# Rongjiehuang/FastDiff

Measured on AMD Instinct MI355X. Metric: real-time factor (audio-sec/wall-sec), N=4 reverse steps, 80x864 mel, higher is better.
Workload: dtype f32 results; 2-piece fp16 operands (22 bit) on fp16 MFMA, fp32 accumulate; GEMM as Winograd F(2,3); exact-fp32 twin; 1 GPU; BASELINE configs[1]: LJSpeech shape, batch=8 x 80x864 mel per GPU, N=4, HIP kernels + hipGraph sampler; batch_per_gpu=8, frames=864, reverse_steps=4, graph=True, weights=random init seed 1234 (no checkpoint offline), world_size=1, gpus_visible=1, oversubscribed=False

## Files before the change

fastdiff_amd/csrc/fd_kernels_kp.hip:

```cpp
#include "fd_kernels_common.h"

namespace fdk_fast {

constexpr int KPF_VALID = 48, KPF_LDI = 68, KPF_LDH = 66;

struct KpFrontW {
    const float *in_pack[fd::NBLK], *in_b[fd::NBLK];
    const float *res_pack[fd::NBLK][6], *res_b[fd::NBLK][6];
};

__global__ void __launch_bounds__(256, 2) k_kp_front(const float *__restrict__ mel, float *__restrict__ hout, KpFrontW w,
                                                     const float *__restrict__ noise, const StepParams *params, int sampler,
                                                     int B, int T, const int *__restrict__ run_if, const int *__restrict__ lens)
{
    __shared__ float xin[fd::COND * KPF_LDI];
    if (run_if && *run_if == 0) return;
    __shared__ float h0[fd::HID * KPF_LDH];
    __shared__ float hA[fd::HID * KPF_LDH];
    __shared__ float hB[fd::HID * KPF_LDH];
    const int blk = blockIdx.z, b = blockIdx.y, t0 = blockIdx.x * KPF_VALID;
    const int Tb = frames_of(lens, b, T);
    if (t0 >= Tb) return;
    const int tid = threadIdx.x, lane = tid & 63, wave = tid >> 6, l31 = lane & 31, hi = lane >> 5;
    const int mt = wave & 1, nt = wave >> 1;
    const int step = sampler ? params->step_idx : 0;
    const float *nz = noise + (((int64_t)step * (sampler > 1 ? B / sampler : B) + b) * fd::NBLK + blk) * fd::COND;
    {
        constexpr int TOTAL = fd::COND * KPF_LDI, NK = (TOTAL + 255) / 256;
        float v[NK];
        const float *src = mel + (int64_t)b * fd::COND * T;
#pragma unroll
        for (int k = 0; k < NK; ++k) {
            const int idx = k * 256 + tid, ci = idx / KPF_LDI, cc = idx - ci * KPF_LDI, t = t0 - 10 + cc;
            v[k] = (idx < TOTAL && t >= 0 && t < Tb) ? src[(int64_t)ci * T + t] + nz[ci] : 0.0f;
        }
#pragma unroll
        for (int k = 0; k < NK; ++k) {
            const int idx = k * 256 + tid;
            if (idx < TOTAL) xin[idx] = v[k];
        }
        if (tid < 128) {
            const int row = tid >> 1, col = (tid & 1) ? KPF_LDH - 1 : 0;
            h0[row * KPF_LDH + col] = 0.0f; hA[row * KPF_LDH + col] = 0.0f; hB[row * KPF_LDH + col] = 0.0f;
        }
    }
    __syncthreads();
    const int c = nt * 32 + l31;
    const int t = t0 - 8 + c;
    const bool inside = (t >= 0 && t < Tb);
    {
        const float4 *pa = reinterpret_cast<const float4 *>(w.in_pack[blk]) + (int64_t)mt * 50 * 64 + lane;
        f32x16 acc;
#pragma unroll
        for (int r = 0; r < 16; ++r) acc[r] = w.in_b[blk][mt * 32 + drow(r, hi)];
#pragma unroll 5
        for (int s4 = 0; s4 < 50; ++s4) {
            const float4 a4 = pa[s4 * 64];
#pragma unroll
            for (int r = 0; r < 4; ++r) {
                const int kk = 8 * s4 + 2 * r, tap = kk / fd::COND, ci = kk % fd::COND + hi;
                acc = mfma32(f4c(a4, r), xin[ci * KPF_LDI + c + tap], acc);
            }
        }
#pragma unroll
        for (int r = 0; r < 16; ++r) h0[(mt * 32 + drow(r, hi)) * KPF_LDH + c + 1] = inside ? lrelu(acc[r], 0.1f) : 0.0f;
    }
    __syncthreads();
    const float *src = h0;
#pragma unroll 1
    for (int l = 0; l < 6; ++l) {
        float *dst = (l & 1) ? hB : hA;
        const float4 *pa = reinterpret_cast<const float4 *>(w.res_pack[blk][l]) + (int64_t)mt * 24 * 64 + lane;
        float4 wa[24];
#pragma unroll
        for (int i = 0; i < 24; ++i) wa[i] = pa[i * 64];
        f32x16 acc;
#pragma unroll
        for (int r = 0; r < 16; ++r) acc[r] = w.res_b[blk][l][mt * 32 + drow(r, hi)];
#pragma unroll
        for (int s = 0; s < 96; ++s) {
            const int tap = s >> 5, ci = ((2 * s) & 63) + hi;
            acc = mfma32(f4c(wa[s >> 2], s & 3), src[ci * KPF_LDH + c + tap], acc);
        }
        if (l < 5) {
#pragma unroll
            for (int r = 0; r < 16; ++r) dst[(mt * 32 + drow(r, hi)) * KPF_LDH + c + 1] = inside ? lrelu(acc[r], 0.1f) : 0.0f;
            __syncthreads();
            src = dst;
        } else if (inside && c >= 8 && c < 8 + KPF_VALID) {
#pragma unroll
            for (int r = 0; r < 16; ++r) {
                const int o = mt * 32 + drow(r, hi);
                hout[(((int64_t)blk * B + b) * fd::HID + o) * T + t] = lrelu(acc[r], 0.1f) + h0[o * KPF_LDH + c + 1];
            }
        }
    }
}

constexpr int KPF_XROW = 336;

struct KpFrontW2 {
    const float4 *in_pack[fd::NBLK];
    const float *in_b[fd::NBLK];
    const float4 *res_pack[fd::NBLK][6];
    const float *res_b[fd::NBLK][6];
};

__device__ __forceinline__ int kpf_off(int row, int slot) { return row * 256 + ((slot ^ (row & 15)) << 4); }

__global__ void __launch_bounds__(256, 2) k_kp_front_h2(const float *__restrict__ mel, float *__restrict__ hout, char *__restrict__ himg,
                                                        KpFrontW2 w, const float *__restrict__ noise, const StepParams *params, int sampler,
                                                        int B, int T, int R, int *__restrict__ range_flags, const int *__restrict__ lens)
{
    __shared__ __attribute__((aligned(16))) char xin[68 * KPF_XROW];
    __shared__ __attribute__((aligned(16))) char hA[66 * 256];
    __shared__ __attribute__((aligned(16))) char hB[66 * 256];
    const int blk = blockIdx.z, b = blockIdx.y, t0 = blockIdx.x * KPF_VALID;
    const int Tb = frames_of(lens, b, T);
    if (range_flags[32 + 19] | range_flags[32]) {
        if (blockIdx.x == 0 && blockIdx.y == 0 && blockIdx.z == 0 && threadIdx.x == 0) { atomicOr(range_flags + 19, 1); atomicOr(range_flags, 1); }
        return;
    }
    if (t0 > Tb) return;
    const int tid = threadIdx.x, lane = tid & 63, wave = tid >> 6, l31 = lane & 31, hi = lane >> 5;
    const int mt = wave & 1, nt = wave >> 1;
    const int step = sampler ? params->step_idx : 0;
    const float *nz = noise + (((int64_t)step * (sampler > 1 ? B / sampler : B) + b) * fd::NBLK + blk) * fd::COND;
    float mx = 0.0f;
    {
        const float *src = mel + (int64_t)b * fd::COND * T;
        float v[3][8];
#pragma unroll
        for (int k = 0; k < 3; ++k) {
            const int u = k * 256 + tid, cg = u / 68, cc = u - cg * 68, t = t0 - 10 + cc;
            const bool ok = u < 680 && t >= 0 && t < Tb;
#pragma unroll
            for (int c = 0; c < 8; ++c) v[k][c] = ok ? src[(int64_t)(cg * 8 + c) * T + t] + nz[cg * 8 + c] : 0.0f;
        }
#pragma unroll
        for (int k = 0; k < 3; ++k) {
            const int u = k * 256 + tid, cg = u / 68, cc = u - cg * 68;
            if (u < 680) {
#pragma unroll
                for (int c = 0; c < 8; ++c) mx = fmaxf(mx, fabsf(v[k][c]));
                float4 ph, pl;
                split8(v[k], ph, pl);
                *reinterpret_cast<float4 *>(xin + cc * KPF_XROW + cg * 16) = ph;
                *reinterpret_cast<float4 *>(xin + cc * KPF_XROW + 160 + cg * 16) = pl;
            }
        }
        if (tid < 64) {
            const int row = (tid & 32) ? 65 : 0, part = tid & 15;
            char *img = (tid & 16) ? hB : hA;
            *reinterpret_cast<float4 *>(img + row * 256 + part * 16) = make_float4(0.f, 0.f, 0.f, 0.f);
        }
    }
    __syncthreads();
    const int c = nt * 32 + l31;
    const int t = t0 - 8 + c;
    const bool inside = (t >= 0 && t < Tb);
    float h0v[16];
    auto store_act = [&](char *img, const f32x16 &ah, const f32x16 &al, float *keep) {
        const int row = c + 1;
#pragma unroll
        for (int j = 0; j < 4; ++j) {
            float v[4];
#pragma unroll
            for (int i = 0; i < 4; ++i) {
                v[i] = inside ? lrelu(fmaf(al[4 * j + i], GX_INV_SCALE, ah[4 * j + i]), 0.1f) : 0.0f;
                mx = fmaxf(mx, fabsf(v[i]));
                if (keep) keep[4 * j + i] = v[i];
            }
            uint2 ph, pl;
            split2(v[0], v[1], ph.x, pl.x);
            split2(v[2], v[3], ph.y, pl.y);
            *reinterpret_cast<uint2 *>(img + kpf_off(row, mt * 4 + j) + 8 * hi) = ph;
            *reinterpret_cast<uint2 *>(img + kpf_off(row, 8 + mt * 4 + j) + 8 * hi) = pl;
        }
    };
    {
        const float4 *pa = w.in_pack[blk] + (int64_t)mt * 2 * 25 * 64 + lane;
        f32x16 ah, al;
#pragma unroll
        for (int r = 0; r < 16; ++r) { ah[r] = w.in_b[blk][mt * 32 + drow(r, hi)]; al[r] = 0.0f; }
        const char *xb = xin + c * KPF_XROW + hi * 16;
#pragma unroll 5
        for (int kg = 0; kg < 25; ++kg) {
            const float4 w1 = pa[kg * 64], w2 = pa[(25 + kg) * 64];
            const int tap = (16 * kg) / fd::COND, o = ((16 * kg) % fd::COND) / 8;
            const float4 b1 = *reinterpret_cast<const float4 *>(xb + tap * KPF_XROW + o * 16);
            const float4 b2 = *reinterpret_cast<const float4 *>(xb + tap * KPF_XROW + 160 + o * 16);
            ah = mfma_f16(w1, b1, ah);
            al = mfma_f16(w1, b2, al);
            al = mfma_f16(w2, b1, al);
        }
        store_act(hA, ah, al, h0v);
    }
    __syncthreads();
    int off[3][2][4];
#pragma unroll
    for (int tap = 0; tap < 3; ++tap)
#pragma unroll
        for (int p = 0; p < 2; ++p)
#pragma unroll
            for (int k4 = 0; k4 < 4; ++k4) off[tap][p][k4] = kpf_off(c + tap, p * 8 + k4 * 2 + hi);
    float4 wa[2][12];
    auto load_w = [&](int l) {
        const float4 *pa = w.res_pack[blk][l] + (int64_t)mt * 2 * 12 * 64 + lane;
#pragma unroll
        for (int p = 0; p < 2; ++p)
#pragma unroll
            for (int kg = 0; kg < 12; ++kg) wa[p][kg] = pa[(p * 12 + kg) * 64];
    };
    load_w(0);
#pragma unroll 1
    for (int l = 0; l < 6; ++l) {
        const char *src = (l & 1) ? hB : hA;
        char *dst = (l & 1) ? hA : hB;
        f32x16 ah, al;
#pragma unroll
        for (int r = 0; r < 16; ++r) { ah[r] = w.res_b[blk][l][mt * 32 + drow(r, hi)]; al[r] = 0.0f; }
#pragma unroll
        for (int kg = 0; kg < 12; ++kg) {
            const float4 b1 = *reinterpret_cast<const float4 *>(src + off[kg >> 2][0][kg & 3]);
            const float4 b2 = *reinterpret_cast<const float4 *>(src + off[kg >> 2][1][kg & 3]);
            ah = mfma_f16(wa[0][kg], b1, ah);
            al = mfma_f16(wa[0][kg], b2, al);
            al = mfma_f16(wa[1][kg], b1, al);
        }
        __builtin_amdgcn_sched_barrier(0);
        if (l < 5) load_w(l + 1);
        __builtin_amdgcn_sched_barrier(0);
        if (l < 5) {
            store_act(dst, ah, al, nullptr);
            __syncthreads();
        } else if (t >= 0 && t < T && c >= 8 && c < 8 + KPF_VALID) {
            char *irow = himg + (((int64_t)blk * B + b) * R + (t + 1)) * 256;
            const int sw = (t + 1) & 15;
#pragma unroll
            for (int j = 0; j < 4; ++j) {
                float v[4];
#pragma unroll
                for (int i = 0; i < 4; ++i) {
                    const int r = 4 * j + i;
                    v[i] = inside ? lrelu(fmaf(al[r], GX_INV_SCALE, ah[r]), 0.1f) + h0v[r] : 0.0f;
                    mx = fmaxf(mx, fabsf(v[i]));
                    hout[(((int64_t)blk * B + b) * fd::HID + mt * 32 + drow(r, hi)) * T + t] = v[i];
                }
                if (himg) {
                    uint2 ph, pl;
                    split2(v[0], v[1], ph.x, pl.x);
                    split2(v[2], v[3], ph.y, pl.y);
                    *reinterpret_cast<uint2 *>(irow + (((mt * 4 + j) ^ sw) << 4) + 8 * hi) = ph;
                    *reinterpret_cast<uint2 *>(irow + (((8 + mt * 4 + j) ^ sw) << 4) + 8 * hi) = pl;
                }
            }
        }
    }
    if (himg) {
        char *ib = himg + ((int64_t)blk * B + b) * R * 256;
        if (blockIdx.x == 0 && tid < 16) *reinterpret_cast<float4 *>(ib + tid * 16) = make_float4(0.f, 0.f, 0.f, 0.f);
        if (blockIdx.x == gridDim.x - 1)
            for (int e = tid; e < (R - 1 - T) * 16; e += 256) *reinterpret_cast<float4 *>(ib + (T + 1) * 256 + e * 16) = make_float4(0.f, 0.f, 0.f, 0.f);
    }
    if (!(mx < GX_LIMIT)) { atomicOr(range_flags + 19, 1); atomicOr(range_flags, 1); }
}

constexpr int GEMM_CT = 4;
constexpr int GEMM_LDH = GEMM_CT * 32 + 4;
constexpr int GEMM_NCOLS = GEMM_CT * 32 + 2;
constexpr int GEMM_NK = (fd::HID * GEMM_NCOLS + 255) / 256;

#ifdef FD_GEMM_TIMING
__device__ long long fd_gdbg[64 * 4 * 4];
#endif

__global__ void __launch_bounds__(256, 2) k_kp_gemm(const float *__restrict__ h , float *__restrict__ kpack,
                                                    const float *g0, const float *g1, const float *g2, const float *gb0,
                                                    const float *gb1, const float *gb2, int B, int T, int chunks_per_utt,
                                                    int chunk_tiles, int n_items, const int *__restrict__ run_if, const int *__restrict__ lens)
{
    __shared__ float hs[2][fd::HID * GEMM_LDH];
    if (run_if && *run_if == 0) return;
    const int tid = threadIdx.x, lane = tid & 63, wave = tid >> 6, l31 = lane & 31, hi = lane >> 5;
    constexpr int XG = fd::KREC / 128;
    const int ny = B * chunks_per_utt;
    const int i0 = (int)((int64_t)blockIdx.x * n_items / gridDim.x), i1 = (int)((int64_t)(blockIdx.x + 1) * n_items / gridDim.x);
    if (i0 >= i1) return;

    struct Item { int blk, xg, b, t_begin; };
    auto decode = [&](int id) {
        Item it;
        it.blk = id / (XG * ny);
        const int rem = id - it.blk * (XG * ny);
        it.xg = rem / ny;
        const int yy = rem - it.xg * ny;
        it.b = yy / chunks_per_utt;
        it.t_begin = (yy - it.b * chunks_per_utt) * chunk_tiles * 32;
        return it;
    };
    float v[33];
    const int scol = tid & 127, srow = tid >> 7;
#define FD_GEMM_FETCH(it)                                                                                              \
    do {                                                                                                               \
        const float *hb__ = h + (((int64_t)(it).blk * B + (it).b) * fd::HID + srow) * T + ((it).t_begin - 1);          \
        const bool ok__ = ((it).t_begin - 1 + scol) >= 0 && ((it).t_begin - 1 + scol) < frames_of(lens, (it).b, T);    \
        _Pragma("unroll") for (int j = 0; j < 32; ++j) v[j] = ok__ ? hb__[(int64_t)(2 * j) * T + scol] : 0.0f;         \
        const int t2__ = (it).t_begin + 127 + (tid & 1);               \
        v[32] = (tid < 128 && t2__ < frames_of(lens, (it).b, T)) ? hb__[(int64_t)((tid >> 1) - srow) * T + 128 + (tid & 1)] : 0.0f;                \
    } while (0)
#define FD_GEMM_COMMIT(bufi)                                                                                           \
    do {                                                                                                               \
        float *hd__ = hs[bufi] + srow * GEMM_LDH + scol;                                                               \
        _Pragma("unroll") for (int j = 0; j < 32; ++j) hd__[2 * j * GEMM_LDH] = v[j];                                   \
        if (tid < 128) hs[bufi][(tid >> 1) * GEMM_LDH + 128 + (tid & 1)] = v[32];                                       \
    } while (0)

    Item cur = decode(i0);
    FD_GEMM_FETCH(cur);
    FD_GEMM_COMMIT(0);
    __syncthreads();
    float4 wb[24];
    float bias = 0.0f;
    int have_blk = -1, have_xg = -1, buf = 0;
#pragma unroll 1
    for (int i = i0; i < i1; ++i) {
        if (cur.blk != have_blk || cur.xg != have_xg) {
            const float *gp = cur.blk == 0 ? g0 : (cur.blk == 1 ? g1 : g2);
            const float *gb = cur.blk == 0 ? gb0 : (cur.blk == 1 ? gb1 : gb2);
            const int ptile = cur.xg * 4 + wave;
#pragma unroll
            for (int k = 0; k < 24; ++k) wb[k] = reinterpret_cast<const float4 *>(gp)[((int64_t)ptile * 24 + k) * 64 + lane];
            bias = gb[ptile * 32 + l31];
            have_blk = cur.blk; have_xg = cur.xg;
        }
        Item nxt = cur;
        const bool more = (i + 1 < i1);
        if (more) { nxt = decode(i + 1); FD_GEMM_FETCH(nxt); }
        const int Tb = frames_of(lens, cur.b, T);
        const int n_frames = min(Tb - cur.t_begin, chunk_tiles * 32);
        const int n_tiles = (n_frames + 31) >> 5;
        float *kout = kpack + ((int64_t)cur.blk * B + cur.b) * T * fd::KREC + (cur.xg * 4 + wave) * 32 + l31;
#pragma unroll 1
        for (int tile = 0; tile < n_tiles; ++tile) {
            f32x16 acc;
#pragma unroll
            for (int r = 0; r < 16; ++r) acc[r] = bias;
            const int hc = hi * GEMM_LDH + l31 + tile * 32;
            const int ho3[3] = {opaque(hc), opaque(hc + 1), opaque(hc + 2)};
#pragma unroll
            for (int s = 0; s < 96; ++s) {
                const int tap = s >> 5, c2 = (2 * s) & 63;
                acc = mfma32(hs[buf][ho3[tap] + c2 * GEMM_LDH], f4c(wb[s >> 2], s & 3), acc);
            }
            const int t0 = cur.t_begin + tile * 32;
            const unsigned base = (unsigned)(t0 + 4 * hi) * (unsigned)fd::KREC;
#ifdef FD_GX_NO_STORE
            if (acc[0] != 12345.678f) continue;
#endif
            if (t0 + 32 <= Tb) {
#pragma unroll
                for (int r = 0; r < 16; ++r) kout[base + (unsigned)(((r & 3) + 8 * (r >> 2)) * fd::KREC)] = acc[r];
            } else {
#pragma unroll
                for (int r = 0; r < 16; ++r)
                    if (t0 + drow(r, hi) < Tb) kout[base + (unsigned)(((r & 3) + 8 * (r >> 2)) * fd::KREC)] = acc[r];
            }
        }
        if (more) FD_GEMM_COMMIT(buf ^ 1);
        __syncthreads();
        buf ^= 1;
        cur = nxt;
    }
}

constexpr int GX_ROWS = GX_CT * 32 + 2;
constexpr int GX_WINB = GX_ROWS * GX_ROWB;
constexpr int GX_NDMA = (GX_WINB + 4095) / 4096;
constexpr int GX_BUFB = GX_NDMA * 4096;
#ifndef FD_GX_STORE_AUX
#define FD_GX_STORE_AUX 2
#endif


__global__ void __launch_bounds__(256) k_h_split(const float *__restrict__ h, unsigned *__restrict__ hx, int *__restrict__ range_flag,
                                                 int B, int T, int R, const int *__restrict__ lens)
{
    const int bb = blockIdx.y;
    const int e = blockIdx.x * 256 + threadIdx.x, cp = e / R, row = e - cp * R;
    if (cp >= 32) return;
    if (range_flag[32] != 0) {
        if (e == 0 && bb == 0) atomicOr(range_flag, 1);
        return;
    }
    const int t = row - 1;
    const bool ok = t >= 0 && t < frames_of(lens, bb % B, T);
    const float *hb = h + (int64_t)bb * fd::HID * T;
    const float a = ok ? hb[(int64_t)(2 * cp) * T + t] : 0.0f, b2 = ok ? hb[(int64_t)(2 * cp + 1) * T + t] : 0.0f;
    if (!(fmaxf(fabsf(a), fabsf(b2)) < GX_LIMIT)) atomicOr(range_flag, 1);
    const _Float16 a1 = (_Float16)a, b1 = (_Float16)b2;
    const _Float16 a2 = (_Float16)((a - (float)a1) * GX_SCALE), b3 = (_Float16)((b2 - (float)b1) * GX_SCALE);
    union { _Float16 h[2]; unsigned u; } p1, p2;
    p1.h[0] = a1; p1.h[1] = b1;
    p2.h[0] = a2; p2.h[1] = b3;
    unsigned *dst = hx + ((int64_t)bb * R + row) * 64 + (cp & 3);
    const unsigned sw = (unsigned)row & 15u, slot = (unsigned)cp >> 2;
    dst[((slot ^ sw) << 2)] = p1.u;
    dst[(((slot + 8u) ^ sw) << 2)] = p2.u;
}

typedef __attribute__((address_space(3))) void *lds_ptr_t;

struct GxItem { int blk, xg, b, chunk; };

struct GxWalk {
    static constexpr int XG = fd::KREC / 128;
    int B, chunks, ny, n_wg, w, q, base, r0, r1;
    int n_mine, left0;
    __device__ __forceinline__ GxWalk(int B_, int chunks_per_utt, int n_items, int n_wg_, int w_)
        : B(B_), chunks(chunks_per_utt), ny(B_ * chunks_per_utt), n_wg(n_wg_), w(w_)
    {
        q = (fd::NBLK * XG) / n_wg; base = q * n_wg * ny;
        const int rest = n_items - base;
        r0 = (int)((int64_t)w * rest / n_wg); r1 = (int)((int64_t)(w + 1) * rest / n_wg);
        n_mine = q * ny + (r1 - r0);
        left0 = (q > 0) ? ny : (r1 - r0);
    }
    __device__ __forceinline__ GxItem decode(int id) const
    {
        GxItem it;
        it.blk = id / (XG * ny);
        const int rem = id - it.blk * (XG * ny);
        it.xg = rem / ny;
        const int yy = rem - it.xg * ny;
        it.b = yy / chunks;
        it.chunk = yy - it.b * chunks;
        return it;
    }
    __device__ __forceinline__ GxItem first() const { return decode((q > 0) ? w * ny : base + r0); }
    __device__ __forceinline__ GxItem advance(GxItem it) const
    {
        if (++it.chunk == chunks) {
            it.chunk = 0;
            if (++it.b == B) {
                it.b = 0;
                if (++it.xg == XG) { it.xg = 0; ++it.blk; }
            }
        }
        return it;
    }
};
#define GX_WALK_NEXT(walk, cur, more, nxt, run, left)                                                                  \
    GxItem nxt = cur;                                                                                                  \
    if (more) {                                                                                                        \
        if (left > 1) nxt = (walk).advance(cur);                                                                       \
        else {                                                  \
            ++run;                                                                                                     \
            nxt = (walk).decode(run < (walk).q ? (run * (walk).n_wg + (walk).w) * (walk).ny : (walk).base + (walk).r0); \
            left = (run < (walk).q ? (walk).ny : (walk).r1 - (walk).r0) + 1;                                           \
        }                                                                                                              \
    }                                                                                                                  \
    --left

template <int ROUNDS, bool PARTIAL_LAST>
__device__ __forceinline__ void gx_window_dma(const char *src , char *lds_buf, int wave_u, int lane)
{
    const unsigned dst = (unsigned)(uintptr_t)(lds_ptr_t)(lds_buf + wave_u * 1024);
    const unsigned voff = lane * 16;
    unsigned keep;
#pragma unroll
    for (int j = 0; j < ROUNDS; ++j) {
        if (PARTIAL_LAST && j == ROUNDS - 1 && wave_u != 0) break;
        asm volatile("s_mov_b32 %0, m0\n\ts_mov_b32 m0, %3\n\ts_nop 0\n\tglobal_load_lds_dwordx4 %1, %2\n\ts_mov_b32 m0, %0"
                     : "=&s"(keep)
                     : "v"(voff), "s"(src + j * 4096), "s"(dst + j * 4096)
                     : "memory");
    }
}

__device__ __forceinline__ void gx_dma(const char *hx, char *lds_buf, const GxItem &it, int B, int R, int wave_u, int lane)
{
#ifndef FD_GX_NO_FETCH
    gx_window_dma<GX_NDMA, true>(hx + (((int64_t)it.blk * B + it.b) * R + it.chunk * (GX_CT * 32)) * GX_ROWB + wave_u * 1024, lds_buf, wave_u, lane);
#endif
}

#ifdef FD_GX_TIMING
__device__ long long fd_gxdbg[8];
#define GX_STAMP(k) do { const long long t__ = __builtin_amdgcn_s_memtime(); ph[k] += t__ - tl; tl = t__; } while (0)
#define GX_TIMING_ARGS , long long (&ph)[8], long long &tl
#define GX_TIMING_PASS , ph, tl
#else
#define GX_STAMP(k) do { } while (0)
#define GX_TIMING_ARGS
#define GX_TIMING_PASS
#endif
template <int BUF, bool FULL>
__device__ __forceinline__ void gx_item(char *lds, const GxItem &cur, bool more, const GxItem &nxt, const char *hx, float *kpack,
                                        const float4 (&wq)[2][12], const f32x16 &bias_lo, const int (&aoff)[2][12], int B, int T, int R,
                                        int wave_u, int lane, int Tb GX_TIMING_ARGS)
{
    const int l31 = lane & 31, hi = lane >> 5;
    GX_STAMP(0);
    if (more) gx_dma(hx, lds + (BUF ^ 1) * GX_BUFB, nxt, B, R, wave_u, lane);
    GX_STAMP(1);
    const int t_begin = cur.chunk * (GX_CT * 32);
    float *krow = kpack + (((int64_t)cur.blk * B + cur.b) * T + t_begin) * fd::KREC + (cur.xg * 4 + wave_u) * 32;
    const unsigned loff = (unsigned)(4 * hi) * (unsigned)fd::KREC + (unsigned)l31;
    const __amdgpu_buffer_rsrc_t rs = __builtin_amdgcn_make_buffer_rsrc(krow, 0, GX_CT * 32 * fd::KREC * 4, 0x00020000);
    const int n_tiles = max(0, min(GX_CT, (Tb - t_begin + 31) >> 5));
    const f32x16 zero = {0.f, 0.f, 0.f, 0.f, 0.f, 0.f, 0.f, 0.f, 0.f, 0.f, 0.f, 0.f, 0.f, 0.f, 0.f, 0.f};
#pragma unroll
    for (int tile = 0; tile < GX_CT; ++tile) {
        if (tile >= n_tiles) break;
        const char *hb = lds + BUF * GX_BUFB + tile * 32 * GX_ROWB;
        f32x16 acc, lo;
        float4 a1 = *reinterpret_cast<const float4 *>(hb + aoff[0][0]), a2 = *reinterpret_cast<const float4 *>(hb + aoff[1][0]);
#pragma unroll
        for (int kg = 0; kg < 12; ++kg) {
            float4 n1 = a1, n2 = a2;
            if (kg + 1 < 12) {
                n1 = *reinterpret_cast<const float4 *>(hb + aoff[0][kg + 1]);
                n2 = *reinterpret_cast<const float4 *>(hb + aoff[1][kg + 1]);
            }
            acc = mfma_f16(a1, wq[0][kg], kg == 0 ? zero : acc);
            lo = mfma_f16(a2, wq[0][kg], kg == 0 ? bias_lo : lo);
#ifndef FD_GX_PROBE_TWO_MFMA
            lo = mfma_f16(a1, wq[1][kg], lo);
#endif
            a1 = n1;
            a2 = n2;
        }
        GX_STAMP(2);
#ifdef FD_GX_NO_STORE
        if (acc[0] != 12345.678f) continue;
#endif
        if (FULL) {
#ifdef FD_GX_STORE_AUX_B0
            if (cur.blk == 0) {
#pragma unroll
                for (int r = 0; r < 16; ++r)
                    __builtin_amdgcn_raw_buffer_store_b32(__float_as_uint(fmaf(lo[r], GX_INV_SCALE, acc[r])), rs, loff * 4u,
                                                          (tile * 32 + (r & 3) + 8 * (r >> 2)) * fd::KREC * 4, FD_GX_STORE_AUX_B0);
            } else
#endif
#pragma unroll
            for (int r = 0; r < 16; ++r)
                __builtin_amdgcn_raw_buffer_store_b32(__float_as_uint(fmaf(lo[r], GX_INV_SCALE, acc[r])), rs, loff * 4u,
                                                      (tile * 32 + (r & 3) + 8 * (r >> 2)) * fd::KREC * 4, FD_GX_STORE_AUX);
        } else {
            float *kt = krow + (int64_t)tile * 32 * fd::KREC;
#pragma unroll
            for (int r = 0; r < 16; ++r)
                if (t_begin + tile * 32 + drow(r, hi) < Tb)
                    (kt + ((r & 3) + 8 * (r >> 2)) * fd::KREC)[loff] = fmaf(lo[r], GX_INV_SCALE, acc[r]);
        }
        GX_STAMP(3);
    }
    if (more) {
        if (FULL && n_tiles == 4) asm volatile("s_waitcnt vmcnt(63)" ::: "memory");
        else if (FULL && n_tiles == 3) asm volatile("s_waitcnt vmcnt(48)" ::: "memory");
        else if (FULL && n_tiles == 2) asm volatile("s_waitcnt vmcnt(32)" ::: "memory");
        else if (FULL && n_tiles == 1) asm volatile("s_waitcnt vmcnt(16)" ::: "memory");
        else asm volatile("s_waitcnt vmcnt(0)" ::: "memory");
    }
    GX_STAMP(4);
    __builtin_amdgcn_s_barrier();
    GX_STAMP(5);
}

__global__ void __launch_bounds__(256, 2) k_kp_gemm_h2(const char *__restrict__ hx , float *__restrict__ kpack,
                                                       const float4 *g0, const float4 *g1, const float4 *g2, const float *gb0,
                                                       const float *gb1, const float *gb2, const int *__restrict__ range_flag, int B,
                                                       int T, int R, int chunks_per_utt, int n_items, const int *__restrict__ lens)
{
    __shared__ __attribute__((aligned(16))) char lds[2 * GX_BUFB];
    const int tid = threadIdx.x, lane = tid & 63, l31 = lane & 31, hi = lane >> 5;
    const int wave_u = __builtin_amdgcn_readfirstlane(tid >> 6);
    if (*range_flag != 0) return;

    GxWalk walk(B, chunks_per_utt, n_items, gridDim.x, blockIdx.x);
    const int n_mine = walk.n_mine;
    if (n_mine <= 0) return;
    int run = 0, left = walk.left0;
    GxItem cur = walk.first();

    int aoff[2][12];
#pragma unroll
    for (int q = 0; q < 2; ++q)
#pragma unroll
        for (int tap = 0; tap < 3; ++tap)
#pragma unroll
            for (int k4 = 0; k4 < 4; ++k4) {
                const int row = l31 + tap;
                aoff[q][tap * 4 + k4] = row * GX_ROWB + (((q * 8 + k4 * 2 + hi) ^ (row & 15)) << 4);
            }

    gx_dma(hx, lds, cur, B, R, wave_u, lane);
    asm volatile("s_waitcnt vmcnt(0)" ::: "memory");
    __builtin_amdgcn_s_barrier();

#ifdef FD_GX_TIMING
    long long ph[8] = {0, 0, 0, 0, 0, 0, 0, 0}, tl = __builtin_amdgcn_s_memtime();
    const long long t_start = tl, r_start = __builtin_amdgcn_s_memrealtime();
#endif
    float4 wq[2][12];
    f32x16 bias_lo;
    int have_blk = -1, have_xg = -1;
#pragma unroll 1
    for (int i = 0; i < n_mine; i += 2) {
#pragma unroll
        for (int half = 0; half < 2; ++half) {
            if (half == 1 && i + 1 >= n_mine) break;
            if (cur.blk != have_blk || cur.xg != have_xg) {
                const float4 *gp = cur.blk == 0 ? g0 : (cur.blk == 1 ? g1 : g2);
                const float *gb = cur.blk == 0 ? gb0 : (cur.blk == 1 ? gb1 : gb2);
                const int ptile = cur.xg * 4 + wave_u;
#pragma unroll
                for (int q2 = 0; q2 < 2; ++q2)
#pragma unroll
                    for (int kg = 0; kg < 12; ++kg) wq[q2][kg] = gp[(((int64_t)ptile * 2 + q2) * 12 + kg) * 64 + lane];
                const float bv = gb[ptile * 32 + l31] * GX_SCALE;
#pragma unroll
                for (int r = 0; r < 16; ++r) bias_lo[r] = bv;
                have_blk = cur.blk; have_xg = cur.xg;
                __builtin_amdgcn_s_waitcnt(0x0F70);
            }
            const bool more = (i + half + 1 < n_mine);
            GX_WALK_NEXT(walk, cur, more, nxt, run, left);
            const int Tb = frames_of(lens, cur.b, T);
            const bool full = (Tb % 32 == 0) || (cur.chunk * (GX_CT * 32) + GX_CT * 32 <= Tb);
            if (half == 0) {
                if (full) gx_item<0, true>(lds, cur, more, nxt, hx, kpack, wq, bias_lo, aoff, B, T, R, wave_u, lane, Tb GX_TIMING_PASS);
                else gx_item<0, false>(lds, cur, more, nxt, hx, kpack, wq, bias_lo, aoff, B, T, R, wave_u, lane, Tb GX_TIMING_PASS);
            } else {
                if (full) gx_item<1, true>(lds, cur, more, nxt, hx, kpack, wq, bias_lo, aoff, B, T, R, wave_u, lane, Tb GX_TIMING_PASS);
                else gx_item<1, false>(lds, cur, more, nxt, hx, kpack, wq, bias_lo, aoff, B, T, R, wave_u, lane, Tb GX_TIMING_PASS);
            }
            cur = nxt;
        }
    }
#ifdef FD_GX_TIMING
    ph[6] = __builtin_amdgcn_s_memtime() - t_start;
    ph[7] = __builtin_amdgcn_s_memrealtime() - r_start;
    if (lane == 0)
        for (int k = 0; k < 8; ++k) atomicAdd((unsigned long long *)&fd_gxdbg[k], (unsigned long long)ph[k]);
#endif
}

constexpr int GW_WINB = GW_PAIRS * GW_ROWB;

__global__ void __launch_bounds__(256) k_h_wino(const float *__restrict__ h, char *__restrict__ wx, int *__restrict__ range_flag, int B, int T,
                                                int P, const int *__restrict__ lens)
{
    const int bb = blockIdx.y;
    const int e = blockIdx.x * 256 + threadIdx.x, p = e >> 3, g = e & 7;
    if (p >= P) return;
    if (range_flag[32] != 0) {
        if (e == 0 && bb == 0) atomicOr(range_flag, 1);
        return;
    }
    const int Tb = frames_of(lens, bb % B, T);
    const float *hb = h + ((int64_t)bb * fd::HID + 8 * g) * T;
    const int t1 = 2 * p;
    float d[8][4];
#pragma unroll
    for (int c = 0; c < 8; ++c) {
        const float *hc = hb + (int64_t)c * T;
        d[c][0] = (t1 - 1 >= 0 && t1 - 1 < Tb) ? hc[t1 - 1] : 0.0f;
        d[c][1] = (t1 < Tb) ? hc[t1] : 0.0f;
        d[c][2] = (t1 + 1 < Tb) ? hc[t1 + 1] : 0.0f;
        d[c][3] = (t1 + 2 < Tb) ? hc[t1 + 2] : 0.0f;
    }
    float mx = 0.0f;
    char *row = wx + ((int64_t)bb * P + p) * GW_ROWB;
    const int sw = p & 15;
#pragma unroll
    for (int j = 0; j < 4; ++j) {
        float u[8];
#pragma unroll
        for (int c = 0; c < 8; ++c) {
            u[c] = j == 0 ? d[c][0] - d[c][2] : (j == 1 ? d[c][1] + d[c][2] : (j == 2 ? d[c][2] - d[c][1] : d[c][1] - d[c][3]));
            mx = fmaxf(mx, fabsf(u[c]));
        }
        float4 ph, pl;
        split8(u, ph, pl);
        *reinterpret_cast<float4 *>(row + j * 256 + ((g ^ sw) << 4)) = ph;
        *reinterpret_cast<float4 *>(row + j * 256 + (((g + 8) ^ sw) << 4)) = pl;
    }
    if (!(mx < GX_LIMIT)) atomicOr(range_flag, 1);
}

__device__ __forceinline__ void gw_dma(const char *wx, char *lds_buf, const GxItem &it, int B, int P, int wave_u, int lane)
{
#ifndef FD_GW_NO_FETCH
    gx_window_dma<GW_WINB / 4096, false>(wx + (((int64_t)it.blk * B + it.b) * P + it.chunk * GW_PAIRS) * GW_ROWB + wave_u * 1024, lds_buf, wave_u, lane);
#endif
}

template <int BUF, bool FULL>
__device__ __forceinline__ void gw_item(char *lds, const GxItem &cur, bool more, const GxItem &nxt, const char *wx, float *kpack,
                                        const float4 (&wq)[2][16], float bias_lo, const int (&aoff)[2][4], int B, int T, int P,
                                        int wave_u, int lane, int Tb)
{
    const int l31 = lane & 31, hi = lane >> 5;
    if (more) gw_dma(wx, lds + (BUF ^ 1) * GW_WINB, nxt, B, P, wave_u, lane);
    const int t_begin = cur.chunk * (2 * GW_PAIRS);
    float *krow = kpack + (((int64_t)cur.blk * B + cur.b) * T + t_begin) * fd::KREC + (cur.xg * 4 + wave_u) * 32;
    const unsigned loff = (unsigned)(8 * hi) * (unsigned)fd::KREC + (unsigned)l31;
    const __amdgpu_buffer_rsrc_t rs = __builtin_amdgcn_make_buffer_rsrc(krow, 0, 2 * GW_PAIRS * fd::KREC * 4, 0x00020000);
    const f32x16 zero = {0.f, 0.f, 0.f, 0.f, 0.f, 0.f, 0.f, 0.f, 0.f, 0.f, 0.f, 0.f, 0.f, 0.f, 0.f, 0.f};
    const char *hb = lds + BUF * GW_WINB;
    constexpr int ORDER[4] = {1, 2, 0, 3};
    f32x16 keep, acc, lo;
#pragma unroll
    for (int r = 0; r < 16; ++r) lo[r] = bias_lo;
    float4 a1, a2;
    auto store16 = [&](int odd) {
#ifdef FD_GX_NO_STORE
        if (FULL) {
#pragma unroll
            for (int r = 0; r < 16; ++r) { const float v_ = fmaf(lo[r], GX_INV_SCALE, acc[r]); asm volatile("" :: "v"(v_)); }
            (void)rs; (void)loff;
            return;
        }
#endif
        if (FULL) {
#pragma unroll
            for (int r = 0; r < 16; ++r) {
                acc[r] = fmaf(lo[r], GX_INV_SCALE, acc[r]);
                __builtin_amdgcn_raw_buffer_store_b32(__float_as_uint(acc[r]), rs, loff * 4u, (2 * ((r & 3) + 8 * (r >> 2)) + odd) * fd::KREC * 4,
                                                      FD_GX_STORE_AUX);
            }
        } else {
#pragma unroll
            for (int r = 0; r < 16; ++r)
                if (t_begin + 2 * drow(r, hi) + odd < Tb) (krow + (2 * ((r & 3) + 8 * (r >> 2)) + odd) * fd::KREC)[loff] = fmaf(lo[r], GX_INV_SCALE, acc[r]);
        }
    };
#pragma unroll
    for (int s = 0; s < 4; ++s) {
        const int j = ORDER[s];
        a1 = *reinterpret_cast<const float4 *>(hb + aoff[0][0] + j * 256);
        a2 = *reinterpret_cast<const float4 *>(hb + aoff[1][0] + j * 256);
#pragma unroll
        for (int k4 = 0; k4 < 4; ++k4) {
            const int kg = j * 4 + k4;
            float4 n1 = a1, n2 = a2;
            if (k4 + 1 < 4) {
                n1 = *reinterpret_cast<const float4 *>(hb + aoff[0][k4 + 1] + j * 256);
                n2 = *reinterpret_cast<const float4 *>(hb + aoff[1][k4 + 1] + j * 256);
            }
            acc = mfma_f16(a1, wq[0][kg], (k4 == 0 && s == 0) ? zero : ((k4 == 0 && s == 3) ? keep : acc));
            lo = mfma_f16(a2, wq[0][kg], (k4 == 0 && s == 3) ? zero : lo);
            lo = mfma_f16(a1, wq[1][kg], lo);
            a1 = n1;
            a2 = n2;
        }
        if (s == 0) {
#pragma unroll
            for (int r = 0; r < 16; ++r) keep[r] = fmaf(lo[r], GX_INV_SCALE, acc[r]);
        } else if (s == 1) {
#pragma unroll
            for (int r = 0; r < 16; ++r) keep[r] = fmaf(2.0f, keep[r], -fmaf(lo[r], GX_INV_SCALE, acc[r]));
        } else store16(s == 3 ? 1 : 0);
    }
    if (more) {
#ifdef FD_GX_NO_STORE
        asm volatile("s_waitcnt vmcnt(0)" ::: "memory");
#else
        if (FULL) asm volatile("s_waitcnt vmcnt(32)" ::: "memory");
        else asm volatile("s_waitcnt vmcnt(0)" ::: "memory");
#endif
    }
    __builtin_amdgcn_s_barrier();
}

typedef float gw_f4 __attribute__((ext_vector_type(4)));
__device__ __forceinline__ gw_f4 mfma16_f16(const float4 &a, const float4 &b, gw_f4 c)
{
    union { float4 f; f16x8 h; } ua, ub;
    ua.f = a;
    ub.f = b;
    return __builtin_amdgcn_mfma_f32_16x16x32_f16(ua.h, ub.h, c, 0, 0, 0);
}
template <int BUF>
__device__ __forceinline__ void gw16_item(char *lds, const GxItem &cur, bool more, const GxItem &nxt, const char *wx, float *kpack,
                                          const float4 (&wq)[2][16] , const float (&bias_lo)[2],
                                          const int (&aoff)[2][2], int B, int T, int P, int wave_u, int lane, int Tb)
{
    if (more) gw_dma(wx, lds + (BUF ^ 1) * GW_WINB, nxt, B, P, wave_u, lane);
    const int t_begin = cur.chunk * (2 * GW_PAIRS);
    float *krow = kpack + (((int64_t)cur.blk * B + cur.b) * T + t_begin) * fd::KREC + (cur.xg * 4 + wave_u) * 32;
    const unsigned loff = gw16_st_lane_off(lane);
    const __amdgpu_buffer_rsrc_t rs = __builtin_amdgcn_make_buffer_rsrc(krow, 0, 2 * GW_PAIRS * fd::KREC * 4, 0x00020000);
    const gw_f4 zero = {0.f, 0.f, 0.f, 0.f};
    constexpr int ORDER[4] = {1, 2, 0, 3};
    int n_fast = 0;
    bool counted = true;
#pragma unroll
    for (int rt = 0; rt < 2; ++rt) {
        const int t0 = t_begin + 32 * rt;
        if (t0 >= Tb) continue;
        const bool whole = t0 + 32 <= Tb;
        const char *hb = lds + BUF * GW_WINB + rt * 16 * GW_ROWB;
        gw_f4 acc[2], lo[2], keep[2];
#pragma unroll
        for (int ct = 0; ct < 2; ++ct) lo[ct] = gw_f4{bias_lo[ct], bias_lo[ct], bias_lo[ct], bias_lo[ct]};
        float4 a1 = *reinterpret_cast<const float4 *>(hb + aoff[0][0] + ORDER[0] * 256);
        float4 a2 = *reinterpret_cast<const float4 *>(hb + aoff[1][0] + ORDER[0] * 256);
#ifdef FD_GW16_PIN
        __builtin_amdgcn_sched_group_barrier(0x100, 2, 0);
#endif
#pragma unroll
        for (int step = 0; step < 8; ++step) {
            const int s = step >> 1, ks = step & 1, j = ORDER[s], w = (2 * j + ks) * 2;
            float4 n1 = a1, n2 = a2;
            if (step + 1 < 8) {
                const int jn = ORDER[(step + 1) >> 1], kn = (step + 1) & 1;
                n1 = *reinterpret_cast<const float4 *>(hb + aoff[0][kn] + jn * 256);
                n2 = *reinterpret_cast<const float4 *>(hb + aoff[1][kn] + jn * 256);
            }
            const bool m3 = (step == 6);
            acc[0] = mfma16_f16(a1, wq[0][w], step == 0 ? zero : (m3 ? keep[0] : acc[0]));
            lo[0] = mfma16_f16(a2, wq[0][w], m3 ? zero : lo[0]);
            acc[1] = mfma16_f16(a1, wq[0][w + 1], step == 0 ? zero : (m3 ? keep[1] : acc[1]));
            lo[1] = mfma16_f16(a2, wq[0][w + 1], m3 ? zero : lo[1]);
            lo[0] = mfma16_f16(a1, wq[1][w], lo[0]);
            lo[1] = mfma16_f16(a1, wq[1][w + 1], lo[1]);
            a1 = n1;
            a2 = n2;
#ifdef FD_GW16_PIN
            if (step + 1 < 8) __builtin_amdgcn_sched_group_barrier(0x100, 2, 0);
            __builtin_amdgcn_sched_group_barrier(0x008, 6, 0);
#endif
            if (ks == 0) continue;
            if (s == 0) {
#pragma unroll
                for (int ct = 0; ct < 2; ++ct)
#pragma unroll
                    for (int i = 0; i < 4; ++i) keep[ct][i] = fmaf(lo[ct][i], GX_INV_SCALE, acc[ct][i]);
            } else if (s == 1) {
#pragma unroll
                for (int ct = 0; ct < 2; ++ct)
#pragma unroll
                    for (int i = 0; i < 4; ++i) keep[ct][i] = fmaf(2.0f, keep[ct][i], -fmaf(lo[ct][i], GX_INV_SCALE, acc[ct][i]));
            } else {
                const int odd = s == 3 ? 1 : 0;
                float v[2][4];
#pragma unroll
                for (int ct = 0; ct < 2; ++ct)
#pragma unroll
                    for (int i = 0; i < 4; ++i) v[ct][i] = fmaf(lo[ct][i], GX_INV_SCALE, acc[ct][i]);
                if (whole) {
#pragma unroll
                    for (int i = 0; i < 4; ++i) {
                        const auto x = __builtin_amdgcn_permlane16_swap(__float_as_uint(v[0][i]), __float_as_uint(v[1][i]), false, false);
#pragma unroll
                        for (int part = 0; part < 2; ++part)
                            __builtin_amdgcn_raw_buffer_store_b32(x[part], rs, loff * 4u, gw16_st_row_off(rt, part, i, odd) * 4, FD_GX_STORE_AUX);
                    }
                } else {
#pragma unroll
                    for (int ct = 0; ct < 2; ++ct)
#pragma unroll
                        for (int i = 0; i < 4; ++i) {
                            const int f = 2 * (16 * rt + gw16_d_pair(lane, i)) + odd;
                            if (t_begin + f < Tb) krow[f * fd::KREC + gw16_d_pos(lane, ct)] = v[ct][i];
                        }
                }
            }
        }
        if (whole) ++n_fast;
        else counted = false;
    }
    if (more) {
        if (counted && n_fast == 2) asm volatile("s_waitcnt vmcnt(32)" ::: "memory");
        else if (counted && n_fast == 1) asm volatile("s_waitcnt vmcnt(16)" ::: "memory");
        else asm volatile("s_waitcnt vmcnt(0)" ::: "memory");
    }
    __builtin_amdgcn_s_barrier();
}

#ifdef FD_GW_CLOCK
__device__ long long fd_gwclk[2];
#endif
template <int TILE>
__global__ void __launch_bounds__(256, 2) k_kp_gemm_w(const char *__restrict__ wx , float *__restrict__ kpack,
                                                      const float4 *g0, const float4 *g1, const float4 *g2, const float *gb0,
                                                      const float *gb1, const float *gb2, const int *__restrict__ range_flag, int B,
                                                      int T, int P, int chunks_per_utt, int n_items, const int *__restrict__ lens)
{
    static_assert(TILE == 16 || TILE == 32, "k_kp_gemm_w: 16- or 32-row matrix tiles");
    __shared__ __attribute__((aligned(16))) char lds[2 * GW_WINB];
    const int tid = threadIdx.x, lane = tid & 63, l31 = lane & 31, hi = lane >> 5;
    const int wave_u = __builtin_amdgcn_readfirstlane(tid >> 6);
    if (*range_flag != 0) return;
    GxWalk walk(B, chunks_per_utt, n_items, gridDim.x, blockIdx.x);
    const int n_mine = walk.n_mine;
    if (n_mine <= 0) return;
    int run = 0, left = walk.left0;
    GxItem cur = walk.first();
    constexpr int NOFF = TILE == 16 ? 2 : 4;
    int aoff[2][NOFF];
#pragma unroll
    for (int q2 = 0; q2 < 2; ++q2)
#pragma unroll
        for (int k4 = 0; k4 < NOFF; ++k4)
            aoff[q2][k4] = TILE == 16 ? gw16_a_off(lane, q2, k4) : l31 * GW_ROWB + (((q2 * 8 + k4 * 2 + hi) ^ (l31 & 15)) << 4);
    gw_dma(wx, lds, cur, B, P, wave_u, lane);
    asm volatile("s_waitcnt vmcnt(0)" ::: "memory");
    __builtin_amdgcn_s_barrier();
#ifdef FD_GW_CLOCK
    const long long clk_t0 = __builtin_amdgcn_s_memtime(), clk_r0 = __builtin_amdgcn_s_memrealtime();
#endif
    float4 wq[2][16];
    float bias_lo[2] = {0.0f, 0.0f};
    int have_blk = -1, have_xg = -1;
#pragma unroll 1
    for (int i = 0; i < n_mine; i += 2) {
#pragma unroll
        for (int half = 0; half < 2; ++half) {
            if (half == 1 && i + 1 >= n_mine) break;
            if (cur.blk != have_blk || cur.xg != have_xg) {
                const float4 *gp = cur.blk == 0 ? g0 : (cur.blk == 1 ? g1 : g2);
                const float *gb = cur.blk == 0 ? gb0 : (cur.blk == 1 ? gb1 : gb2);
                const int ptile = cur.xg * 4 + wave_u;
                if constexpr (TILE == 16) {
#pragma unroll
                    for (int q2 = 0; q2 < 2; ++q2)
#pragma unroll
                        for (int jk = 0; jk < 8; ++jk)
#pragma unroll
                            for (int ct = 0; ct < 2; ++ct) wq[q2][jk * 2 + ct] = gp[gw16_b_idx(ptile, q2, jk >> 1, jk & 1, ct, lane)];
#pragma unroll
                    for (int ct = 0; ct < 2; ++ct) bias_lo[ct] = gb[ptile * 32 + gw16_d_pos(lane, ct)] * GX_SCALE;
                } else {
#pragma unroll
                    for (int q2 = 0; q2 < 2; ++q2)
#pragma unroll
                        for (int kg = 0; kg < 16; ++kg) wq[q2][kg] = gp[(((int64_t)ptile * 2 + q2) * 16 + kg) * 64 + lane];
                    bias_lo[0] = gb[ptile * 32 + l31] * GX_SCALE;
                }
                have_blk = cur.blk; have_xg = cur.xg;
                __builtin_amdgcn_s_waitcnt(0x0F70);
            }
            const bool more = (i + half + 1 < n_mine);
            GX_WALK_NEXT(walk, cur, more, nxt, run, left);
            const int Tb = frames_of(lens, cur.b, T);
            if constexpr (TILE == 16) {
                if (half == 0) gw16_item<0>(lds, cur, more, nxt, wx, kpack, wq, bias_lo, aoff, B, T, P, wave_u, lane, Tb);
                else gw16_item<1>(lds, cur, more, nxt, wx, kpack, wq, bias_lo, aoff, B, T, P, wave_u, lane, Tb);
            } else {
                const bool full = cur.chunk * (2 * GW_PAIRS) + 2 * GW_PAIRS <= Tb;
                if (half == 0) {
                    if (full) gw_item<0, true>(lds, cur, more, nxt, wx, kpack, wq, bias_lo[0], aoff, B, T, P, wave_u, lane, Tb);
                    else gw_item<0, false>(lds, cur, more, nxt, wx, kpack, wq, bias_lo[0], aoff, B, T, P, wave_u, lane, Tb);
                } else {
                    if (full) gw_item<1, true>(lds, cur, more, nxt, wx, kpack, wq, bias_lo[0], aoff, B, T, P, wave_u, lane, Tb);
                    else gw_item<1, false>(lds, cur, more, nxt, wx, kpack, wq, bias_lo[0], aoff, B, T, P, wave_u, lane, Tb);
                }
            }
            cur = nxt;
        }
    }
#ifdef FD_GW_CLOCK
    if (tid == 0) {
        atomicAdd((unsigned long long *)&fd_gwclk[0], (unsigned long long)(__builtin_amdgcn_s_memtime() - clk_t0));
        atomicAdd((unsigned long long *)&fd_gwclk[1], (unsigned long long)(__builtin_amdgcn_s_memrealtime() - clk_r0));
    }
#endif
}

}

namespace fdk {
using namespace fdk_fast;

hipError_t fast_kp_front(const Launch &L, const StepIO &io, int B, int T)
{
    fd_context *c = L.ctx;
    const DevWeights &w = c->w;
    const dim3 grid((T + KPF_VALID - 1) / KPF_VALID, B, fd::NBLK);
    const StepMode &m = *L.mode;
    const int *lens = m.ragged ? c->ws.lens_dev : nullptr;
    const int *run_if = nullptr;
    const char *name = "kp_front";
    const Pipe pipe = fd_pipe(m, m.conv_f16 && w.kpf_f16_ok, 19);
    if (pipe != PIPE_F32_ONLY) {
        KpFrontW2 k2;
        for (int n = 0; n < fd::NBLK; ++n) {
            k2.in_pack[n] = reinterpret_cast<const float4 *>(w.kp_in_h2[n]); k2.in_b[n] = w.blk[n].kp_in.b;
            for (int l = 0; l < 6; ++l) { k2.res_pack[n][l] = reinterpret_cast<const float4 *>(w.kp_res_h2[n][l]); k2.res_b[n][l] = w.blk[n].kp_res[l].b; }
        }
        const bool image = front_writes_h_image(m, w);
        FD_LAUNCH(L, name, k_kp_front_h2, grid, dim3(256), 0, io.mel, c->ws.kp_hB, image ? reinterpret_cast<char *>(c->ws.h_f16) : (char *)nullptr, k2,
                  (const float *)c->ws.noise, (const StepParams *)c->ws.params, io.sampler, B, T, gx_rows(T), c->ws.range_flag, lens);
        run_if = c->ws.range_flag + 19;
        name = "kp_front_fp32_fallback";
        if (pipe == PIPE_F16_ONLY) return hipSuccess;
    }
    KpFrontW kw;
    for (int n = 0; n < fd::NBLK; ++n) {
        kw.in_pack[n] = w.kp_in_pack[n]; kw.in_b[n] = w.blk[n].kp_in.b;
        for (int l = 0; l < 6; ++l) { kw.res_pack[n][l] = w.kp_res_pack[n][l]; kw.res_b[n][l] = w.blk[n].kp_res[l].b; }
    }
    FD_LAUNCH(L, name, k_kp_front, grid, dim3(256), 0, io.mel, c->ws.kp_hB, kw, (const float *)c->ws.noise,
              (const StepParams *)c->ws.params, io.sampler, B, T, run_if, lens);
    return hipSuccess;
}

struct GemmGrid { int chunks, items, grid; };
static GemmGrid gemm_grid(const fd_context *c, int B, int chunks)
{
    const int items = fd::NBLK * (fd::KREC / 128) * B * chunks;
    return {chunks, items, items < 2 * c->num_cus ? items : 2 * c->num_cus};
}

hipError_t fast_kp_gemm(const Launch &L, int B, int T)
{
    fd_context *c = L.ctx;
    const DevWeights &w = c->w;
    const StepMode &m = *L.mode;
    const int *lens = m.ragged ? c->ws.lens_dev : nullptr;
    const Pipe pipe = fd_pipe(m, m.gemm_f16 && w.gemm_f16_ok, 0);
    const bool f16 = pipe != PIPE_F32_ONLY;
    if (f16 && m.gemm_wino && w.gemm_w_ok) {
        const int P = gw_pairs(T);
        const GemmGrid g = gemm_grid(c, B, P / GW_PAIRS);
        FD_LAUNCH(L, "h_wino", k_h_wino, dim3((8 * P + 255) / 256, fd::NBLK * B), dim3(256), 0, (const float *)c->ws.kp_hB,
                  reinterpret_cast<char *>(c->ws.h_f16), c->ws.range_flag, B, T, P, lens);
        const auto gemm_w = m.gemm_tile16 ? &k_kp_gemm_w<16> : &k_kp_gemm_w<32>;
        FD_LAUNCH(L, "kp_gemm_f16x2", gemm_w, dim3(g.grid), dim3(256), 0,
                  reinterpret_cast<const char *>(c->ws.h_f16), c->ws.kpack,
                  reinterpret_cast<const float4 *>(w.gemm_w_pack[0]), reinterpret_cast<const float4 *>(w.gemm_w_pack[1]),
                  reinterpret_cast<const float4 *>(w.gemm_w_pack[2]), w.gemm_bias[0], w.gemm_bias[1], w.gemm_bias[2],
                  (const int *)c->ws.range_flag, B, T, P, g.chunks, g.items, lens);
        if (pipe == PIPE_F16_ONLY) return hipSuccess;
    } else if (f16) {
        const int R = gx_rows(T);
        const GemmGrid g = gemm_grid(c, B, (T + GX_CT * 32 - 1) / (GX_CT * 32));
        if (!front_writes_h_image(m, w))
            FD_LAUNCH(L, "h_split", k_h_split, dim3((32 * R + 255) / 256, fd::NBLK * B), dim3(256), 0, (const float *)c->ws.kp_hB,
                      reinterpret_cast<unsigned *>(c->ws.h_f16), c->ws.range_flag, B, T, R, lens);
        FD_LAUNCH(L, "kp_gemm_f16x2", k_kp_gemm_h2, dim3(g.grid), dim3(256), 0, reinterpret_cast<const char *>(c->ws.h_f16), c->ws.kpack,
                  reinterpret_cast<const float4 *>(w.gemm_h2_pack[0]), reinterpret_cast<const float4 *>(w.gemm_h2_pack[1]),
                  reinterpret_cast<const float4 *>(w.gemm_h2_pack[2]), w.gemm_bias[0], w.gemm_bias[1], w.gemm_bias[2],
                  (const int *)c->ws.range_flag, B, T, R, g.chunks, g.items, lens);
        if (pipe == PIPE_F16_ONLY) return hipSuccess;
    }
    const int tiles_per_utt = (T + 31) / 32;
    const GemmGrid g = gemm_grid(c, B, (tiles_per_utt + GEMM_CT - 1) / GEMM_CT);
    const int chunk_tiles = (tiles_per_utt + g.chunks - 1) / g.chunks;
    FD_LAUNCH(L, f16 ? "kp_gemm_fp32_fallback" : "kp_gemm", k_kp_gemm, dim3(g.grid), dim3(256), 0, (const float *)c->ws.kp_hB, c->ws.kpack,
              w.gemm_pack[0], w.gemm_pack[1], w.gemm_pack[2], w.gemm_bias[0], w.gemm_bias[1], w.gemm_bias[2], B, T, g.chunks,
              chunk_tiles, g.items, f16 ? (const int *)c->ws.range_flag : (const int *)nullptr, lens);
    return hipSuccess;
}

}
```

Measured before the change: 10210 x real-time.

## Split Winograd MFMA accumulator chains and pack epilogue FMAs in gw16 kernel

Adds a compile-time GW16_CHAIN mask, default 9 (bits 1 and 8). Bit 1 stores the bias as a full vector tile and injects it into the first lo MFMA instead of pre-initialising lo. Bit 8 hides the lane id behind an empty asm so the tail-store index math is not rematerialised. The SURVIVE (second accumulator chain) and packed-FMA paths are off by default, so the active change is mainly register and scheduling tweaks that cost extra VGPRs for the vector bias.

Result: no change. 10210 x real-time, median of 3 (-0.0%).

```diff
diff --git a/fastdiff_amd/csrc/fd_kernels_kp.hip b/fastdiff_amd/csrc/fd_kernels_kp.hip
--- a/fastdiff_amd/csrc/fd_kernels_kp.hip
+++ b/fastdiff_amd/csrc/fd_kernels_kp.hip
@@ -776,7 +776,13 @@
     __builtin_amdgcn_s_barrier();
 }
 
+#ifdef FD_GW16_CHAIN
+constexpr int GW16_CHAIN = FD_GW16_CHAIN;
+#else
+constexpr int GW16_CHAIN = 9;
+#endif
 typedef float gw_f4 __attribute__((ext_vector_type(4)));
+typedef float gw_f2 __attribute__((ext_vector_type(2)));
 __device__ __forceinline__ gw_f4 mfma16_f16(const float4 &a, const float4 &b, gw_f4 c)
 {
     union { float4 f; f16x8 h; } ua, ub;
@@ -784,11 +790,38 @@
     ub.f = b;
     return __builtin_amdgcn_mfma_f32_16x16x32_f16(ua.h, ub.h, c, 0, 0, 0);
 }
+template <bool NEG = false>
+__device__ __forceinline__ gw_f4 gw16_fma(gw_f4 a, gw_f4 b, gw_f4 c)
+{
+    if constexpr ((GW16_CHAIN & 4) != 0) {
+        const gw_f2 cl = c.lo;
+        const gw_f2 l = __builtin_elementwise_fma(a.lo, b.lo, NEG ? -cl : cl);
+        if (NEG) return gw_f4{l.x, l.y, fmaf(a[2], b[2], -c[2]), fmaf(a[3], b[3], -c[3])};
+        const gw_f2 h = __builtin_elementwise_fma(a.hi, b.hi, c.hi);
+        return gw_f4{l.x, l.y, h.x, h.y};
+    } else {
+        gw_f4 r;
+#pragma unroll
+        for (int i = 0; i < 4; ++i) r[i] = fmaf(a[i], b[i], NEG ? -c[i] : c[i]);
+        return r;
+    }
+}
+typedef std::conditional_t<(GW16_CHAIN & 1) != 0, gw_f4, float> gw16_bias_t;
+__device__ __forceinline__ gw_f4 gw16_bias_tile(const gw_f4 &b) { return b; }
+__device__ __forceinline__ gw_f4 gw16_bias_tile(float b) { return gw_f4{b, b, b, b}; }
+template <typename T>
+__device__ __forceinline__ T gw16_bias_make(float b)
+{
+    if constexpr (std::is_same_v<T, float>) return b;
+    else return T{b, b, b, b};
+}
 template <int BUF>
 __device__ __forceinline__ void gw16_item(char *lds, const GxItem &cur, bool more, const GxItem &nxt, const char *wx, float *kpack,
-                                          const float4 (&wq)[2][16] , const float (&bias_lo)[2],
+                                          const float4 (&wq)[2][16] , const gw16_bias_t (&bias_lo)[2],
                                           const int (&aoff)[2][2], int B, int T, int P, int wave_u, int lane, int Tb)
 {
+    constexpr bool SURVIVE = (GW16_CHAIN & 2) != 0;
+    const gw_f4 two = {2.0f, 2.0f, 2.0f, 2.0f}, inv = {GX_INV_SCALE, GX_INV_SCALE, GX_INV_SCALE, GX_INV_SCALE};
     if (more) gw_dma(wx, lds + (BUF ^ 1) * GW_WINB, nxt, B, P, wave_u, lane);
     const int t_begin = cur.chunk * (2 * GW_PAIRS);
     float *krow = kpack + (((int64_t)cur.blk * B + cur.b) * T + t_begin) * fd::KREC + (cur.xg * 4 + wave_u) * 32;
@@ -804,9 +837,11 @@
         if (t0 >= Tb) continue;
         const bool whole = t0 + 32 <= Tb;
         const char *hb = lds + BUF * GW_WINB + rt * 16 * GW_ROWB;
-        gw_f4 acc[2], lo[2], keep[2];
-#pragma unroll
-        for (int ct = 0; ct < 2; ++ct) lo[ct] = gw_f4{bias_lo[ct], bias_lo[ct], bias_lo[ct], bias_lo[ct]};
+        gw_f4 acc[2], lo[2], acc2[2], lo2[2], keep[2];
+        if constexpr (!(GW16_CHAIN & 1)) {
+#pragma unroll
+            for (int ct = 0; ct < 2; ++ct) lo[ct] = gw16_bias_tile(bias_lo[ct]);
+        }
         float4 a1 = *reinterpret_cast<const float4 *>(hb + aoff[0][0] + ORDER[0] * 256);
         float4 a2 = *reinterpret_cast<const float4 *>(hb + aoff[1][0] + ORDER[0] * 256);
 #ifdef FD_GW16_PIN
@@ -821,13 +856,24 @@
                 n1 = *reinterpret_cast<const float4 *>(hb + aoff[0][kn] + jn * 256);
                 n2 = *reinterpret_cast<const float4 *>(hb + aoff[1][kn] + jn * 256);
             }
-            const bool m3 = (step == 6);
-            acc[0] = mfma16_f16(a1, wq[0][w], step == 0 ? zero : (m3 ? keep[0] : acc[0]));
-            lo[0] = mfma16_f16(a2, wq[0][w], m3 ? zero : lo[0]);
-            acc[1] = mfma16_f16(a1, wq[0][w + 1], step == 0 ? zero : (m3 ? keep[1] : acc[1]));
-            lo[1] = mfma16_f16(a2, wq[0][w + 1], m3 ? zero : lo[1]);
-            lo[0] = mfma16_f16(a1, wq[1][w], lo[0]);
-            lo[1] = mfma16_f16(a1, wq[1][w + 1], lo[1]);
+            if (SURVIVE && (s == 1 || s == 2)) {
+                const bool m2 = (step == 2);
+                acc2[0] = mfma16_f16(a1, wq[0][w], m2 ? acc[0] : acc2[0]);
+                lo2[0] = mfma16_f16(a2, wq[0][w], m2 ? lo[0] : lo2[0]);
+                acc2[1] = mfma16_f16(a1, wq[0][w + 1], m2 ? acc[1] : acc2[1]);
+                lo2[1] = mfma16_f16(a2, wq[0][w + 1], m2 ? lo[1] : lo2[1]);
+                lo2[0] = mfma16_f16(a1, wq[1][w], lo2[0]);
+                lo2[1] = mfma16_f16(a1, wq[1][w + 1], lo2[1]);
+            } else {
+                const bool m3 = (step == 6) && !SURVIVE;
+                const bool b0 = (step == 0) && (GW16_CHAIN & 1);
+                acc[0] = mfma16_f16(a1, wq[0][w], step == 0 ? zero : (m3 ? keep[0] : acc[0]));
+                lo[0] = mfma16_f16(a2, wq[0][w], b0 ? gw16_bias_tile(bias_lo[0]) : (m3 ? zero : lo[0]));
+                acc[1] = mfma16_f16(a1, wq[0][w + 1], step == 0 ? zero : (m3 ? keep[1] : acc[1]));
+                lo[1] = mfma16_f16(a2, wq[0][w + 1], b0 ? gw16_bias_tile(bias_lo[1]) : (m3 ? zero : lo[1]));
+                lo[0] = mfma16_f16(a1, wq[1][w], lo[0]);
+                lo[1] = mfma16_f16(a1, wq[1][w + 1], lo[1]);
+            }
             a1 = n1;
             a2 = n2;
 #ifdef FD_GW16_PIN
@@ -836,22 +882,24 @@
 #endif
             if (ks == 0) continue;
             if (s == 0) {
-#pragma unroll
-                for (int ct = 0; ct < 2; ++ct)
-#pragma unroll
-                    for (int i = 0; i < 4; ++i) keep[ct][i] = fmaf(lo[ct][i], GX_INV_SCALE, acc[ct][i]);
+                if (!SURVIVE) {
+#pragma unroll
+                    for (int ct = 0; ct < 2; ++ct) keep[ct] = gw16_fma(lo[ct], inv, acc[ct]);
+                }
             } else if (s == 1) {
 #pragma unroll
-                for (int ct = 0; ct < 2; ++ct)
-#pragma unroll
-                    for (int i = 0; i < 4; ++i) keep[ct][i] = fmaf(2.0f, keep[ct][i], -fmaf(lo[ct][i], GX_INV_SCALE, acc[ct][i]));
+                for (int ct = 0; ct < 2; ++ct) {
+                    if (SURVIVE) {
+                        acc[ct] = gw16_fma<true>(two, acc[ct], acc2[ct]);
+                        lo[ct] = gw16_fma<true>(two, lo[ct], lo2[ct]);
+                    } else keep[ct] = gw16_fma<true>(two, keep[ct], gw16_fma(lo[ct], inv, acc[ct]));
+                }
             } else {
                 const int odd = s == 3 ? 1 : 0;
-                float v[2][4];
-#pragma unroll
-                for (int ct = 0; ct < 2; ++ct)
-#pragma unroll
-                    for (int i = 0; i < 4; ++i) v[ct][i] = fmaf(lo[ct][i], GX_INV_SCALE, acc[ct][i]);
+                const bool second = SURVIVE && s == 2;
+                gw_f4 v[2];
+#pragma unroll
+                for (int ct = 0; ct < 2; ++ct) v[ct] = second ? gw16_fma(lo2[ct], inv, acc2[ct]) : gw16_fma(lo[ct], inv, acc[ct]);
                 if (whole) {
 #pragma unroll
                     for (int i = 0; i < 4; ++i) {
@@ -861,12 +909,14 @@
                             __builtin_amdgcn_raw_buffer_store_b32(x[part], rs, loff * 4u, gw16_st_row_off(rt, part, i, odd) * 4, FD_GX_STORE_AUX);
                     }
                 } else {
+                    int ln = lane;
+                    if constexpr ((GW16_CHAIN & 8) != 0) asm volatile("" : "+v"(ln));
 #pragma unroll
                     for (int ct = 0; ct < 2; ++ct)
 #pragma unroll
                         for (int i = 0; i < 4; ++i) {
-                            const int f = 2 * (16 * rt + gw16_d_pair(lane, i)) + odd;
-                            if (t_begin + f < Tb) krow[f * fd::KREC + gw16_d_pos(lane, ct)] = v[ct][i];
+                            const int f = 2 * (16 * rt + gw16_d_pair(ln, i)) + odd;
+                            if (t_begin + f < Tb) krow[f * fd::KREC + gw16_d_pos(ln, ct)] = v[ct][i];
                         }
                 }
             }
@@ -916,6 +966,7 @@
 #endif
     float4 wq[2][16];
     float bias_lo[2] = {0.0f, 0.0f};
+    gw16_bias_t bias16[2] = {gw16_bias_t(), gw16_bias_t()};
     int have_blk = -1, have_xg = -1;
 #pragma unroll 1
     for (int i = 0; i < n_mine; i += 2) {
@@ -934,7 +985,10 @@
 #pragma unroll
                             for (int ct = 0; ct < 2; ++ct) wq[q2][jk * 2 + ct] = gp[gw16_b_idx(ptile, q2, jk >> 1, jk & 1, ct, lane)];
 #pragma unroll
-                    for (int ct = 0; ct < 2; ++ct) bias_lo[ct] = gb[ptile * 32 + gw16_d_pos(lane, ct)] * GX_SCALE;
+                    for (int ct = 0; ct < 2; ++ct) {
+                        const float bv = gb[ptile * 32 + gw16_d_pos(lane, ct)] * GX_SCALE;
+                        bias16[ct] = gw16_bias_make<gw16_bias_t>(bv);
+                    }
                 } else {
 #pragma unroll
                     for (int q2 = 0; q2 < 2; ++q2)
@@ -949,8 +1003,8 @@
             GX_WALK_NEXT(walk, cur, more, nxt, run, left);
             const int Tb = frames_of(lens, cur.b, T);
             if constexpr (TILE == 16) {
-                if (half == 0) gw16_item<0>(lds, cur, more, nxt, wx, kpack, wq, bias_lo, aoff, B, T, P, wave_u, lane, Tb);
-                else gw16_item<1>(lds, cur, more, nxt, wx, kpack, wq, bias_lo, aoff, B, T, P, wave_u, lane, Tb);
+                if (half == 0) gw16_item<0>(lds, cur, more, nxt, wx, kpack, wq, bias16, aoff, B, T, P, wave_u, lane, Tb);
+                else gw16_item<1>(lds, cur, more, nxt, wx, kpack, wq, bias16, aoff, B, T, P, wave_u, lane, Tb);
             } else {
                 const bool full = cur.chunk * (2 * GW_PAIRS) + 2 * GW_PAIRS <= Tb;
                 if (half == 0) {
```
